# JiaoLab2021/varigraph

Measured on AMD Instinct MI355X. Metric: 150 bp reads/sec genotyped (k=27), higher is better.
Workload: dtype u64

## Files before the change

varigraph_amd/csrc/vgmi_api_table.cpp:

```cpp
#include "vgmi_ctx.h"

namespace vgapi {

void layout_image(ImageHeader& h, uint32_t k, uint64_t n_keys)
{
    memset(&h, 0, sizeof h);
    memcpy(h.magic, "VGMITBL1", 8);
    h.k = k;
    h.n_keys = n_keys;
    const bool smallk = k >= 19 && k <= 25 && n_keys <= VG_GRID_LDS_MAX_KEYS && !(getenv("VGMI_SMALLK") && getenv("VGMI_SMALLK")[0] == '0');
    const bool off_k = (getenv("VGMI_CTABLE_K") && getenv("VGMI_CTABLE_K")[0] == '0') || (getenv("VGMI_CTABLE") && getenv("VGMI_CTABLE")[0] == '0') ||
                       (getenv("VGMI_XTABLE") && getenv("VGMI_XTABLE")[0] == '0');
    const bool largek = ((k >= 19 && k <= 25 && n_keys > VG_GRID_LDS_MAX_KEYS) || ((k == 26 || k == 28) && n_keys > 0)) && n_keys < (1ULL << 31) - 16 && !off_k;
    const bool compact = (k == 27 || smallk || largek) && !getenv("VGMI_WIDE_SLOTS");
    h.slot_bytes = compact ? 8 : 16;
    uint64_t cap = 64;
    uint64_t lf_mul = compact ? 8 : 4;
    if (const char* e = getenv("VGMI_TABLE_MUL")) lf_mul = (uint64_t)atoi(e) > 1 ? (uint64_t)atoi(e) : 2;
    while (cap < lf_mul * n_keys) cap <<= 1;
    while (cap > (1ULL << 32) && cap / 2 >= 2 * n_keys) cap >>= 1;
    h.cap = cap;
    h.home_bucket_log2 = 0;
    if (k == 27 && n_keys > VG_GRID_LDS_MAX_KEYS) {
        h.home_bucket_log2 = 5;
// ... 491 lines not shown
                const uint32_t q[4] = {(uint32_t)(lo >> 24) & 0x7FFFFu, (uint32_t)(lo >> 43) & 0x7FFFFu, (uint32_t)hi & 0x7FFFFu, (uint32_t)(hi >> 19) & 0x7FFFFu};
                for (int i = 0; i < 4 && q[0] != 0; ++i) {
                    if (q[i] == 0) continue;
                    for (const uint32_t at : {q[i], flip - q[i]}) {
                        if (at >= Tp || (BKT[at] != VG_PT_NO_BUCKET && BKT[at] != (uint32_t)b)) {
                            never[b] = 1;
                            if (at < Tp) never[BKT[at]] = 1;
                            continue;
                        }
                        BKT[at] = (uint32_t)b;
                    }
                }
            }
        }
        for (uint64_t at = 0; at < Tp; ++at) {
            if (BKT[at] == VG_PT_NO_BUCKET) continue;
            for (uint32_t j = 0; j < W && at + j < Tp; ++j) NEED[BKT[at]] += vb[at + j];
        }
        for (size_t b = 0; b < n_buckets; ++b)
            if (never[b] || NEED[b] == 0) NEED[b] = 0xFFFFFFFFu;
    }
    he = hipMalloc(reinterpret_cast<void**>(&c->d_pt_index), index.size() * 8);
    if (he == hipSuccess) he = hipMalloc(reinterpret_cast<void**>(&c->d_pt_S), S.size() * 4);
    if (he == hipSuccess) he = hipMalloc(reinterpret_cast<void**>(&c->d_pt_VB), VB.size() * 4);
    const size_t pc_words = (size_t)Tp + 64, cnt_words = pt_done ? n_buckets : 0, done_words = pt_done ? (n_buckets + 31) / 32 : 0;
    const size_t live_words = pt_done ? VG_LIVE_WORDS : 0;
    const size_t sb_words = VB.size() + pc_words + cnt_words + done_words + live_words;
    if (he == hipSuccess) he = hipMalloc(reinterpret_cast<void**>(&c->d_pt_SB), sb_words * 4);
    if (pt_done) {
        if (he == hipSuccess) he = hipMalloc(reinterpret_cast<void**>(&c->d_pt_BKT), BKT.size() * 4);
        if (he == hipSuccess) he = hipMalloc(reinterpret_cast<void**>(&c->d_pt_NEED), NEED.size() * 4);
        if (he == hipSuccess) he = hipMemcpy(c->d_pt_BKT, BKT.data(), BKT.size() * 4, hipMemcpyHostToDevice);
        if (he == hipSuccess) he = hipMemcpy(c->d_pt_NEED, NEED.data(), NEED.size() * 4, hipMemcpyHostToDevice);
    }
    if (he == hipSuccess) he = hipMalloc(reinterpret_cast<void**>(&c->d_pt_SLOT), (size_t)(Tp + 64) * 4);
    if (he == hipSuccess) he = hipMemcpy(c->d_pt_index, index.data(), index.size() * 8, hipMemcpyHostToDevice);
    if (he == hipSuccess) he = hipMemcpy(c->d_pt_S, S.data(), S.size() * 4, hipMemcpyHostToDevice);
    if (he == hipSuccess) he = hipMemcpy(c->d_pt_VB, VB.data(), VB.size() * 4, hipMemcpyHostToDevice);
    if (he == hipSuccess) he = hipMemset(c->d_pt_SB, 0, sb_words * 4);
    if (he == hipSuccess) he = hipMemset(c->d_pt_SLOT, 0, (size_t)(Tp + 64) * 4);
    if (he == hipSuccess) he = hipMemcpy(c->d_pt_SLOT, slot.data(), (size_t)Tp * 4, hipMemcpyHostToDevice);
    {
        std::vector<uint32_t> place_of_slot(h.cap, 0u);
        for (uint64_t i = 0; i < n; ++i) place_of_slot[(uint32_t)P[i].y] = (uint32_t)(32 + kpos[i]);
        if (he == hipSuccess) he = hipMalloc(reinterpret_cast<void**>(&c->d_pt_PLACE), h.cap * 4);
        if (he == hipSuccess) he = hipMemcpy(c->d_pt_PLACE, place_of_slot.data(), h.cap * 4, hipMemcpyHostToDevice);
    }
    HIPCHK(c, he);
    c->pt_sb_bytes = sb_words * 4;
    if (getenv("VGMI_VERBOSE"))
        fprintf(stderr, "[vgmi] path table: %llu k-mers in %llu chains, %llu bases, %llu 12-mers with a fifth place, %llu buckets with a third 12-mer\n",
                (unsigned long long)n, (unsigned long long)chains, (unsigned long long)Tp, (unsigned long long)slow_cx, (unsigned long long)bucket_ovf);
    c->tv.pt.index = c->d_pt_index;
    c->tv.pt.S = c->d_pt_S;
    c->tv.pt.VB = c->d_pt_VB;
    c->tv.pt.SB = c->d_pt_SB;
    c->tv.pt.SLOT = c->d_pt_SLOT;
    c->tv.pt.PLACE = c->d_pt_PLACE;
    const char* pcv = getenv("VGMI_PT_POSCOUNT");
    c->tv.pt.PC = pcv && pcv[0] == '0' ? nullptr : c->d_pt_SB + VB.size();
    if (pt_done) {
        c->tv.pt.BKT = c->d_pt_BKT;
        c->tv.pt.NEED = c->d_pt_NEED;
        c->tv.pt.CNT = c->d_pt_SB + VB.size() + pc_words;
        c->tv.pt.DONE = c->tv.pt.CNT + cnt_words;
        c->tv.pt.DONE_N = c->tv.pt.DONE + done_words;
    }
    {
        const char* lv = getenv("VGMI_PT_LIVE");
        const char* lb = getenv("VGMI_PT_LIVE_BYTES");
        const unsigned long long unit = lb ? strtoull(lb, nullptr, 10) : 1ull << 30;
        c->live_unit = unit < 2048 ? 2048 : unit;
        const char* lf = getenv("VGMI_PT_LIVE_FACTOR");
        const int factor = lf ? atoi(lf) : 4;
        c->live_factor = (uint32_t)(factor < 2 ? 2 : factor > 16 ? 16 : factor);
        live_drop(c);
        if (pt_done && !(lv && lv[0] == '0') && c->tv.grid && h.grid_words_log2 == VG_GRID_LDS_WORDS_LOG2) {
            HIPCHK(c, hipMalloc(reinterpret_cast<void**>(&c->d_pt_live), (size_t)VG_LIVE_IMAGES * VG_GRID_LDS_WORDS * 4));
            for (auto& e : c->live_ev) HIPCHK(c, hipEventCreateWithFlags(&e, hipEventDisableTiming));
        }
    }
    c->tv.pt.bucket_log2 = bucket_log2;
    c->tv.pt.Tp = (uint32_t)Tp;
    return VGMI_OK;
}

}

extern "C" {


int vgmi_table_upload(vgmi_ctx* c, const uint64_t* keys, size_t n_keys, uint32_t k)
{
    if (!c) return VGMI_E_INVALID;
    if (k < 1 || k > 28) return fail(c, VGMI_E_INVALID, "k must be in 1..28 (reference assert, kmer.cpp:124)");
    if (n_keys && !keys) return fail(c, VGMI_E_INVALID, "keys is NULL");
    if (n_keys >= (1ULL << 31)) return fail(c, VGMI_E_INVALID, "too many keys");
    HIPCHK(c, hipSetDevice(c->device));
    HIPCHK(c, hipStreamSynchronize(c->stream));
    free_table(c);
    layout_image(c->hdr, k, n_keys);
    c->image_bytes = c->hdr.total_bytes;
    HIPCHK(c, hipMalloc(reinterpret_cast<void**>(&c->d_image), c->image_bytes));
    HIPCHK(c, hipMemsetAsync(c->d_image, 0, c->image_bytes, c->stream));
    HIPCHK(c, hipMemcpyAsync(c->d_image, &c->hdr, sizeof c->hdr, hipMemcpyHostToDevice, c->stream));
    HIPCHK(c, hipMemsetAsync(c->d_status, 0, 4, c->stream));
    int rc = adopt_image(c);
    if (rc) return rc;
    HIPCHK(c, launch_table_clear(c->tv, c->stream));
    uint64_t* d_keys = nullptr;
    if (n_keys) {
        HIPCHK(c, hipMalloc(reinterpret_cast<void**>(&d_keys), n_keys * 8));
        HIPCHK(c, hipMemcpyAsync(d_keys, keys, n_keys * 8, hipMemcpyHostToDevice, c->stream));
        hipError_t e = launch_table_insert(c->tv, d_keys, n_keys, k, c->d_key_slot,
                                           const_cast<uint32_t*>(c->tv.filter), const_cast<uint32_t*>(c->tv.grid),
                                           c->hdr.grid_mer == 12, c->d_status, c->stream);
        if (e != hipSuccess) { (void)hipFree(d_keys); HIPCHK(c, e); }
    }
    hipError_t e = hipStreamSynchronize(c->stream);
    if (d_keys) (void)hipFree(d_keys);
    HIPCHK(c, e);
    rc = check_status(c);
    if (rc) { free_table(c); return rc; }
    rc = build_xtable(c);
    if (rc) { free_table(c); return rc; }
    rc = build_ptable(c);
    if (rc) { free_table(c); return rc; }
    c->read_base = 0;
    return VGMI_OK;
}

int vgmi_table_lookup(vgmi_ctx* c, const uint64_t* keys, size_t n, uint32_t* index_out)
{
    if (!c || (n && (!keys || !index_out))) return VGMI_E_INVALID;
    if (!c->has_table) return fail(c, VGMI_E_STATE, "no table");
    if (n == 0) return VGMI_OK;
    HIPCHK(c, hipSetDevice(c->device));
    const TableView tv = c->tv;
    const uint64_t cap = c->hdr.cap, n_keys = c->hdr.n_keys;
    const size_t chunk = std::min<size_t>(n, (size_t)1 << 25);
    hipStream_t st = nullptr;
    uint32_t* key_of_slot = nullptr;
    uint64_t* d_keys[2] = {nullptr, nullptr};
    uint32_t* d_out[2] = {nullptr, nullptr};
    hipEvent_t done[2] = {nullptr, nullptr};
    hipError_t he = hipStreamCreateWithFlags(&st, hipStreamNonBlocking);
    if (he == hipSuccess && tv.slots8) {
        he = hipMalloc(reinterpret_cast<void**>(&key_of_slot), cap * 4);
        if (he == hipSuccess) he = hipMemsetAsync(key_of_slot, 0xFF, cap * 4, st);
        if (he == hipSuccess) he = launch_table_key_of_slot(c->d_key_slot, n_keys, key_of_slot, st);
    }
    for (int b = 0; b < 2 && he == hipSuccess; ++b) {
        he = hipMalloc(reinterpret_cast<void**>(&d_keys[b]), chunk * 8);
        if (he == hipSuccess) he = hipMalloc(reinterpret_cast<void**>(&d_out[b]), chunk * 4);
        if (he == hipSuccess) he = hipEventCreateWithFlags(&done[b], hipEventDisableTiming);
    }
    size_t at[2] = {0, 0}, len[2] = {0, 0};
    auto collect = [&](int b) {
        if (he != hipSuccess || !len[b]) return;
        he = hipEventSynchronize(done[b]);
        len[b] = 0;
    };
    int b = 0;
    for (size_t off = 0; off < n && he == hipSuccess; off += chunk, b ^= 1) {
        collect(b);
        if (he != hipSuccess) break;
// ... 168 lines not shown
```

varigraph_amd/csrc/vgmi_kernels.h:

```cpp
#ifndef VGMI_KERNELS_H
#define VGMI_KERNELS_H
#include <hip/hip_runtime.h>
#include <stdint.h>

#include "vgmi_bam_filter.h"
#include "vgmi_read_filter.h"
#include "vgmi_count_plan.h"
#include "vgmi_ctable.h"
#include "vgmi_device.h"

#ifdef VGMI_ABLATION
#define VG_DBG(x) (x)
#else
#define VG_DBG(x) 0u
#endif
uint32_t vgmi_dbg_env();

namespace vgk {

enum { K_MODE_COUNT = 0, K_MODE_KEYS = 1, K_MODE_BLOOM = 2, K_MODE_DEBIT = 3 };

#define XT_HOPS 3u
struct XTableView {
    unsigned long long* lines;
    uint32_t n_lines;
    uint32_t tag_bits;
    uint32_t id_shift;
    uint32_t* counts;
    const ulonglong2* over;
    uint32_t over_mask;
    const uint4* cb;
    uint32_t n_buckets;
    uint32_t k;
};

struct PathView {
    const unsigned long long* index;
    const uint32_t* S;
    const uint32_t* VB;
    uint32_t* SB;
    const uint32_t* SLOT;
    const uint32_t* PLACE;
    uint32_t* PC;
    const uint32_t* BKT;
    const uint32_t* NEED;
    uint32_t* CNT;
    uint32_t* DONE;
    uint32_t* DONE_N;
    uint32_t bucket_log2;
    uint32_t Tp;
};
#define VG_PT_NO_BUCKET 0xFFFFFFFFu
#define VG_LIVE_IMAGES 8u
#define VG_LIVE_WORDS (16u + 64u * 16u)
__host__ __device__ inline uint32_t vg_done_n_part(uint32_t bucket) { return 16u + ((bucket & 63u) << 4); }

struct TableView {
    VgSlot* slots;
    unsigned long long* slots8;
    uint64_t cap_mask;
    uint32_t k;
    uint32_t home_bucket_log2;
    uint32_t home_by_offset;
    const uint32_t* filter;
    uint32_t filter_words_log2;
    uint32_t filter_shift;
    const uint32_t* grid;
    uint32_t grid_words_log2;
    uint8_t* sat_dirty;
    XTableView xt;
    PathView pt;
    uint32_t* counts;
};

#define VG_BLOOM_MAX_HASH 32
struct BloomView {
    uint8_t* filter;
    uint64_t m;
    uint64_t magic;
    uint32_t n_hash;
    uint32_t seeds[VG_BLOOM_MAX_HASH];
};

struct RowParams {
    const uint8_t* bases;
    uint64_t n_bytes;
    uint64_t row_begin;
    uint64_t pair_begin;
    uint64_t row_end;
    uint64_t emit_from;
    uint32_t k;
    uint32_t dbg;
    uint32_t* status;
    const unsigned long long* n_bytes_dev;
    uint32_t tail27;
    uint32_t l1_min;
    TableView table;
    uint64_t* keys_out;
    BloomView bloom;
};

struct FqState {
    unsigned long long n_records;
    unsigned long long n_bases;
    unsigned long long consumed;
    unsigned long long packed_bytes;
    unsigned long long n_masked;
    uint32_t stopped;
    uint32_t tail_len;
    uint32_t start;
    uint32_t consumed_end;
    uint32_t n_lines, n_good, first_bad, dirty;
    unsigned long long n_seen;
    unsigned long long n_short, n_long, n_low_fraction, n_low_mean;
    uint32_t rf_dropped;
    uint32_t rf_pad;
};
struct SubParams {
    uint32_t on;
    unsigned long long seed, threshold;
};
struct FqBuffers {
    const uint8_t* raw;
    uint8_t* raw_next;
    uint8_t* packed;
    uint32_t* tile;
    uint32_t* nlpos;
    uint32_t* rec_bytes;
    uint32_t* out_off;
    uint32_t* block_sum;
    FqState* state;
    uint32_t cap_lines, tail_max;
    uint32_t min_qual;
    SubParams sub;
    vgh::ReadFilterParams rf;
};
hipError_t launch_fastq_init(FqState* st, uint32_t tail_max, hipStream_t s);
hipError_t launch_fastq_chunk(const FqBuffers& b, uint32_t n_new, hipStream_t s, const uint32_t* n_new_dev = nullptr);
hipError_t launch_scan_small(uint32_t* v, uint32_t n, uint32_t* total, hipStream_t s);

hipError_t launch_fastq_lines(const FqBuffers& b, uint32_t n_new, hipStream_t s, const uint32_t* n_new_dev = nullptr);

struct FaBuffers {
    FqBuffers q;
    unsigned long long* total;
    unsigned long long* bsum;
    uint32_t* dest;
    uint32_t* rec_d;
    uint32_t* rec_pos;
    unsigned long long* bsum_hdr;
};
// ... 273 lines not shown
```

varigraph_amd/csrc/vgmi_kernels.hip:

```cpp
#include <hip/hip_runtime.h>
#include <stdint.h>

#include "vgmi_device.h"
#include "vgmi_kernels.h"
#include "vgmi_xtable.h"

namespace vgk {

__device__ __forceinline__ uint32_t funnel(uint32_t hi, uint32_t lo, uint32_t sh)
{
    return __builtin_amdgcn_alignbit(hi, lo, sh);
}

__device__ __forceinline__ uint32_t rc_word(uint32_t x)
{
    uint32_t r = __builtin_bitreverse32(x);
    r = ((r >> 1) & 0x55555555u) | ((r & 0x55555555u) << 1);
    return ~r;
}

__device__ __forceinline__ uint64_t mod_u64(uint64_t x, uint64_t m, uint64_t magic)
{
    uint64_t q = __umul64hi(x, magic);
    uint64_t r = x - q * m;
// ... 664 lines not shown
__device__ __forceinline__ uint32_t vm_load_byte_sync(const uint8_t* ptr)
{
    uint32_t v;
    asm volatile("global_load_ubyte %0, %1, off ; VGHOT\n\ts_waitcnt vmcnt(0) ; VGHOT" : "=&v"(v) : "v"(ptr) : "memory");
    return v;
}
__device__ __forceinline__ void vm_atomic_or_sync(uint32_t* ptr, uint32_t bits)
{
    asm volatile("global_atomic_or %0, %1, off ; VGHOT\n\ts_waitcnt vmcnt(0) ; VGHOT" : : "v"(ptr), "v"(bits) : "memory");
}
__device__ __forceinline__ void vm_atomic_add_sync(uint32_t* ptr, uint32_t v)
{
    asm volatile("global_atomic_add %0, %1, off ; VGHOT\n\ts_waitcnt vmcnt(0) ; VGHOT" : : "v"(ptr), "v"(v) : "memory");
}
__device__ __forceinline__ void vm_store_byte_sync(uint8_t* ptr, uint32_t v)
{
    asm volatile("global_store_byte %0, %1, off ; VGHOT\n\ts_waitcnt vmcnt(0) ; VGHOT" : : "v"(ptr), "v"(v) : "memory");
}
template <bool COMPACT>
__device__ __forceinline__ uint4 vm_slot_value()
{
    uint4 v = make_uint4(0u, 0u, 0u, 0u);
    if (COMPACT) asm volatile("v_mov_b32 %0, v124 ; VGHOT\n\tv_mov_b32 %1, v125 ; VGHOT" : "=v"(v.x), "=v"(v.y));
    else asm volatile("v_mov_b32 %0, v124 ; VGHOT\n\tv_mov_b32 %1, v125 ; VGHOT\n\tv_mov_b32 %2, v126 ; VGHOT\n\tv_mov_b32 %3, v127 ; VGHOT"
                      : "=v"(v.x), "=v"(v.y), "=v"(v.z), "=v"(v.w));
    return v;
}
__device__ __forceinline__ uint32_t vm_atomic_old()
{
    uint32_t v;
    asm volatile("v_mov_b32 %0, v123 ; VGHOT" : "=v"(v));
    return v;
}

#define VG_ROW27 768u

#define VG_LUT27_BYTES 4096u
typedef __attribute__((address_space(3))) const uint16_t lds_u16;
typedef __attribute__((address_space(3))) const uint32_t lds_u32;

__device__ __forceinline__ void stage_lut27(uint32_t tid, uint32_t nthreads)
{
    typedef __attribute__((address_space(3))) uint16_t lds_u16_rw;
    for (uint32_t i = tid; i < 2048; i += nthreads) {
        const uint32_t set = i >> 10, b = (i >> 8) & 3u, c = vg_nt4(i & 255u);
        reinterpret_cast<lds_u16_rw*>((uintptr_t)0)[i] =
            (uint16_t)(((c & 3u) << (2 * (3 - b))) | ((c >> 2) << ((set ? 12 : 8) + b)));
    }
}

struct Addr4 { uint32_t a0, a1, a2, a3; };

#define VG_SDWA_X2(REG, B) "v_lshlrev_b32_sdwa %" #B ", %4, " REG " dst_sel:DWORD dst_unused:UNUSED_PAD src0_sel:DWORD src1_sel:BYTE_" #B " ; VGHOT\n\t"
#define VG_SDWA_ROW(REG) asm volatile(VG_SDWA_X2(REG, 0) VG_SDWA_X2(REG, 1) VG_SDWA_X2(REG, 2) VG_SDWA_X2(REG, 3) \
                                      : "=&v"(a.a0), "=&v"(a.a1), "=&v"(a.a2), "=&v"(a.a3) : "v"(one))
template <int R, int D>
__device__ __forceinline__ Addr4 lut_addr4(const uint32_t one)
{
    Addr4 a;
    if (R == 0 && D == 0) VG_SDWA_ROW("v116");
    if (R == 0 && D == 1) VG_SDWA_ROW("v117");
    if (R == 0 && D == 2) VG_SDWA_ROW("v118");
    if (R == 1 && D == 0) VG_SDWA_ROW("v120");
    if (R == 1 && D == 1) VG_SDWA_ROW("v121");
    if (R == 1 && D == 2) VG_SDWA_ROW("v122");
    return a;
}

template <int R, int D>
__device__ __forceinline__ Addr4 luts_addr4(const uint32_t one)
{
    Addr4 a;
    if (R == 0 && D == 0) VG_SDWA_ROW("v116");
    if (R == 0 && D == 1) VG_SDWA_ROW("v117");
    if (R == 0 && D == 2) VG_SDWA_ROW("v118");
    if (R == 0 && D == 3) VG_SDWA_ROW("v119");
    if (R == 1 && D == 0) VG_SDWA_ROW("v120");
    if (R == 1 && D == 1) VG_SDWA_ROW("v121");
    if (R == 1 && D == 2) VG_SDWA_ROW("v122");
    if (R == 1 && D == 3) VG_SDWA_ROW("v123");
    return a;
}

template <int SET>
__device__ __forceinline__ uint32_t encode4(const Addr4& a)
{
    const uint32_t e0 = *reinterpret_cast<lds_u16*>((uintptr_t)(a.a0 + SET * 2048u));
    const uint32_t e1 = *reinterpret_cast<lds_u16*>((uintptr_t)(a.a1 + SET * 2048u + 512u));
    const uint32_t e2 = *reinterpret_cast<lds_u16*>((uintptr_t)(a.a2 + SET * 2048u + 1024u));
    uint32_t e3 = *reinterpret_cast<lds_u16*>((uintptr_t)(a.a3 + SET * 2048u + 1536u));
    asm("" : "+v"(e3));
    return e0 | e1 | e2 | e3;
}

template <bool LDS_BM, bool COMPACT>
__global__ __launch_bounds__(LDS_BM ? 1024 : 256) void count27_kernel(RowParams p)
{
    constexpr uint32_t MASK_HI = (1u << (2 * 27 - 32)) - 1;
    extern __shared__ __attribute__((aligned(16))) uint8_t smem[];
    const uint32_t tid = threadIdx.x;
    const uint32_t lane = tid & 63u;
    const uint32_t wave = tid >> 6;
    const uint32_t nwaves = blockDim.x >> 6;

    typedef uint32_t u32x4 __attribute__((ext_vector_type(4)));
    typedef __attribute__((address_space(3))) u32x4 lds_u4_rw;
    typedef __attribute__((address_space(3))) uint64_t lds_u64_rw;
    const uint32_t wave_u = (uint32_t)__builtin_amdgcn_readfirstlane((int)wave);
    const uint32_t rings0 = VG_LUT27_BYTES + (LDS_BM ? VG_GRID_LDS_WORDS * 4u : 0u);
    const uint32_t runs_base = rings0 + wave_u * (VG_RUNQ * 16u);
    const uint32_t req_base = rings0 + nwaves * (VG_RUNQ * 16u) + wave_u * (VG_REQ * 8u);
    stage_lut27(tid, blockDim.x);
    if (LDS_BM) {
        const uint4* src = reinterpret_cast<const uint4*>(p.table.grid);
        uint4* dst = reinterpret_cast<uint4*>(smem + VG_LUT27_BYTES);
        for (uint32_t i = tid; i < VG_GRID_LDS_WORDS / 4; i += blockDim.x) dst[i] = src[i];
    }
    __syncthreads();
    const uint32_t* g_grid = p.table.grid;
    const uint32_t gwl = LDS_BM ? VG_GRID_LDS_WORDS_LOG2 : p.table.grid_words_log2;
    VgSlot* const slots = p.table.slots;
    unsigned long long* const slots8 = p.table.slots8;
    uint32_t* const counts = p.table.counts;
    const uint64_t cap_mask = p.table.cap_mask;
    const uint32_t hb_log2 = p.table.home_bucket_log2;
    const bool hb_off = p.table.home_by_offset != 0;

    const uint64_t total_pairs = p.n_bytes_dev ? *p.n_bytes_dev / (2 * VG_ROW27) : p.row_end >> 1;
    const uint64_t total_waves = (uint64_t)gridDim.x * nwaves;
    const uint64_t ppw = (total_pairs + total_waves - 1) / total_waves;
    const uint64_t gw = (uint64_t)blockIdx.x * nwaves + wave_u;
    const uint64_t r0v = gw * ppw;
    const uint64_t r1v = r0v + ppw < total_pairs ? r0v + ppw : total_pairs;
    const uint64_t r0 = ((uint64_t)(uint32_t)__builtin_amdgcn_readfirstlane((int)(r0v >> 32)) << 32) |
                        (uint32_t)__builtin_amdgcn_readfirstlane((int)(uint32_t)r0v);
    const uint64_t r1 = ((uint64_t)(uint32_t)__builtin_amdgcn_readfirstlane((int)(r1v >> 32)) << 32) |
                        (uint32_t)__builtin_amdgcn_readfirstlane((int)(uint32_t)r1v);
    if (r0 >= r1) return;
    uint32_t one;
    asm volatile("v_mov_b32 %0, 1" : "=v"(one));
    const uint32_t lane_off = lane * 12u;
    const uint8_t* const bases = p.bases;

    uint32_t pr1_be = 0, pr2_be = 0, pr3_be = 0, pr1_inv = 0xFFFu, pr2_inv = 0xFFFu, pr3_inv = 0xFFFu;
    const uint64_t rs = r0 > 0 ? r0 - 1 : r0;

    uint32_t n_after_row = 0;
    uint32_t n_after_slot = 2;
    uint64_t b_canon = 0, b_slot = 0;
    bool b_active = false;
    uint64_t p_slot = 0;
    bool p_bumped = false;

    const uint32_t my_run = lane / 12u, my_win = lane % 12u;
    const uint32_t my_sh = 2 * (11 - my_win), my_vbit = 12 + my_win;
    uint32_t run_head = 0, run_n = 0, req_head = 0, req_n = 0;
    auto ring_slot = [](uint32_t pos) -> uint32_t {
        const uint32_t w = pos - VG_RUNQ;
        return w < pos ? w : pos;
    };

    auto probe_issue = [&](bool act, uint64_t kmer, uint64_t dist) __attribute__((always_inline)) {
        const uint64_t rc = vg_revcomp(kmer, 27);
        const uint64_t canon = kmer < rc ? kmer : rc;
        b_canon = canon | (dist << 54);
        const uint64_t home = (!LDS_BM && hb_log2) ? vg_thash_local(canon, canon == kmer ? rc : kmer, hb_log2, hb_off) : vg_thash(canon);
// ... 174 lines not shown
        const uint32_t iB1 = lane >= 1 ? b1_inv : a1_inv, iB2 = lane >= 2 ? b2_inv : a2_inv, iB3 = lane >= 3 ? b3_inv : a3_inv;
        pr1_be = b1_be; pr2_be = b2_be; pr3_be = b3_be; pr1_inv = b1_inv; pr2_inv = b2_inv; pr3_inv = b3_inv;
        if (it < n_warm) continue;

        {
            const uint32_t adjA = invA & ((invA << 1) | (iA1 >> 11));
            const uint32_t adjB = invB & ((invB << 1) | (iB1 >> 11));
            if (__builtin_expect(__ballot((adjA | adjB) != 0) != 0, 0)) {
                empty_read_check(adjA, cur);
                empty_read_check(adjB, cur + VG_ROW27);
            }
        }

        const RowScan sa = scan_probe(beA, invA, beA1, beA2, beA3, iA1, iA2, iA3);
        const RowScan sb = scan_probe(beB, invB, beB1, beB2, beB3, iB1, iB2, iB3);
        const uint64_t ballA = __builtin_amdgcn_ballot_w64(sa.ok16 && (sa.gw32 & sa.gm) == sa.gm && sa.vm != 0);
        const uint64_t ballB = __builtin_amdgcn_ballot_w64(sb.ok16 && (sb.gw32 & sb.gm) == sb.gm && sb.vm != 0);
        const uint32_t nA = (uint32_t)__builtin_popcountll(ballA), nB = (uint32_t)__builtin_popcountll(ballB);
        if (VG_DBG(p.dbg) & 1u) continue;
        enqueue(sa, ballA, run_head + run_n);
        run_n += nA;
        while (run_n + nB > VG_RUNQ) drain_step();
        enqueue(sb, ballB, run_head + run_n);
        run_n += nB;
        if (run_n >= VG_RUN_BATCH || req_n >= 32u) drain_step();
        while (run_n >= 3 * VG_RUN_BATCH || req_n >= 48u) drain_step();
    }
    do {
        drain_step();
    } while (run_n != 0 || req_n != 0 || __builtin_amdgcn_ballot_w64(b_active) != 0);
    vm_wait_imm<0>();
}

#define VG_ROW27S 1024u
#define VG_RUN_BATCH_S 4u

template <bool PT, uint32_t K = 27>
__global__ __launch_bounds__(1024) void count27s_kernel(RowParams p)
{
    static_assert(K == 27 || (PT && K >= 19 && K <= 25), "count27s_kernel: k = 27, or the path-table form for k = 19 .. 25 (a run of k + 7 bases is two words)");
    constexpr uint32_t MASK_HI = (1u << (2 * K - 32)) - 1;
    extern __shared__ __attribute__((aligned(16))) uint8_t smem[];
    const uint32_t tid = threadIdx.x;
    const uint32_t lane = tid & 63u;
    const uint32_t wave = tid >> 6;
    const uint32_t nwaves = blockDim.x >> 6;
    typedef uint32_t u32x4 __attribute__((ext_vector_type(4)));
    typedef __attribute__((address_space(3))) u32x4 lds_u4_rw;
    typedef __attribute__((address_space(3))) uint64_t lds_u64_rw;
    const uint32_t wave_u = (uint32_t)__builtin_amdgcn_readfirstlane((int)wave);
    const uint32_t rings0 = VG_LUT27_BYTES + VG_GRID_LDS_WORDS * 4u;
    const uint32_t runs_base = rings0 + wave_u * (VG_RUNQ * 16u);
    const uint32_t req_base = rings0 + nwaves * (VG_RUNQ * 16u) + wave_u * (VG_REQ * 8u);
    stage_lut27(tid, blockDim.x);
    {
        const uint4* src = reinterpret_cast<const uint4*>(p.table.grid);
        uint4* dst = reinterpret_cast<uint4*>(smem + VG_LUT27_BYTES);
        for (uint32_t i = tid; i < VG_GRID_LDS_WORDS / 4; i += blockDim.x) dst[i] = src[i];
    }
    __syncthreads();
    unsigned long long* const slots8 = p.table.slots8;
    uint32_t* const counts = p.table.counts;
    const uint64_t cap_mask = p.table.cap_mask;

    const uint64_t total_pairs = p.n_bytes_dev ? *p.n_bytes_dev / (2 * VG_ROW27S) : p.row_end >> 1;
    const uint64_t pair_begin = p.n_bytes_dev ? 0u : p.pair_begin;
    const uint64_t total_waves = (uint64_t)gridDim.x * nwaves;
    const uint64_t ppw = (total_pairs - pair_begin + total_waves - 1) / total_waves;
    const uint64_t gw = (uint64_t)blockIdx.x * nwaves + wave_u;
    const uint64_t r0v = pair_begin + gw * ppw;
    const uint64_t r1v = r0v + ppw < total_pairs ? r0v + ppw : total_pairs;
    const uint64_t r0 = ((uint64_t)(uint32_t)__builtin_amdgcn_readfirstlane((int)(r0v >> 32)) << 32) |
                        (uint32_t)__builtin_amdgcn_readfirstlane((int)(uint32_t)r0v);
    const uint64_t r1 = ((uint64_t)(uint32_t)__builtin_amdgcn_readfirstlane((int)(r1v >> 32)) << 32) |
                        (uint32_t)__builtin_amdgcn_readfirstlane((int)(uint32_t)r1v);
    if (r0 >= r1) return;
    uint32_t one;
    asm volatile("v_mov_b32 %0, 1" : "=v"(one));
    const uint32_t lane_off = lane * 16u;
    const uint8_t* const bases = p.bases;

    uint32_t pr1_be = 0, pr2_be = 0, pr1_inv = 0xFFFFu, pr2_inv = 0xFFFFu;
    const uint64_t rs = r0 > 0 ? r0 - 1 : r0;

    uint32_t n_after_row = 0, n_after_slot = 2;
    uint64_t b_canon = 0, b_slot = 0;
    bool b_active = false;
    uint64_t p_slot = 0;
    bool p_bumped = false;

    const uint32_t my_run = lane >> 4, my_win = lane & 15u;
    const uint32_t my_sh = 2 * (15 - my_win);
    uint32_t run_head = 0, run_n = 0, req_head = 0, req_n = 0;
    auto ring_slot = [](uint32_t pos) -> uint32_t {
        const uint32_t w = pos - VG_RUNQ;
        return w < pos ? w : pos;
    };

    auto probe_issue = [&](bool act, uint64_t kmer, uint64_t dist) __attribute__((always_inline)) {
        const uint64_t rc = vg_revcomp(kmer, K);
        const uint64_t canon = kmer < rc ? kmer : rc;
        b_canon = canon | (dist << 54);
        b_slot = (vg_thash(canon) + dist) & cap_mask;
        b_active = act;
        if (act) vms_load_slot(&slots8[b_slot]);
        ++n_after_row;
        n_after_slot = 0;
    };
    constexpr uint32_t RQ = 112;
    const uint32_t rq_base = rings0 + wave_u * (VG_RUNQ * 16u + VG_REQ * 8u);
    auto rq_wrap = [](uint32_t pos) -> uint32_t { return pos >= RQ ? pos - RQ : pos; };
    const unsigned long long* const pt_index = p.table.pt.index;
    const uint32_t* const ptS = p.table.pt.S;
    const uint32_t* const ptVB = p.table.pt.VB;
    uint32_t* const ptSB = p.table.pt.SB;
    const uint32_t* const ptSLOT = p.table.pt.SLOT;
    uint32_t* const ptPC = p.table.pt.PC;
    const uint32_t* const ptBKT = p.table.pt.BKT;
    const uint32_t* const ptNEED = p.table.pt.NEED;
    uint32_t* const ptCNT = p.table.pt.CNT;
    uint32_t* const ptDONE_N = p.table.pt.DONE_N;
    uint32_t* const ptDONE = p.table.pt.DONE;
    const uint32_t pt_Tp = p.table.pt.Tp, pt_bshift = 32u - p.table.pt.bucket_log2;
    const uint32_t l1_min = (uint32_t)__builtin_amdgcn_readfirstlane((int)p.l1_min);
    uint32_t n_after_idx = 8, n_after_seq = 8;
    u32x4 l1_run = {0u, 0u, 0u, 0u};
    uint32_t l1_n = 0, l1_phase = 0;
    uint32_t pl[4] = {0u, 0u, 0u, 0u};
    bool l1_slow = false;
    uint32_t l1_done_bit = 0;
    auto hot = [&](uint32_t k) __attribute__((always_inline)) {
        n_after_row += k;
        n_after_idx += k;
        n_after_seq += k;
    };
    auto set_saturated = [&](uint32_t pos, uint32_t mir) __attribute__((always_inline)) -> uint32_t {
        const uint32_t a = vm_atomic_or_ret_sync(ptSB + (pos >> 5), 1u << (pos & 31u));
        const uint32_t b = vm_atomic_or_ret_sync(ptSB + (mir >> 5), 1u << (mir & 31u));
        return ((~a >> (pos & 31u)) & 1u) | (((~b >> (mir & 31u)) & 1u) << 1);
    };
    auto done_events = [&](uint32_t fired, uint32_t pos) __attribute__((always_inline)) {
        constexpr uint32_t W = K == 27 ? 16u : 8u;
        uint64_t ev = __builtin_amdgcn_ballot_w64(fired != 0);
        while (ev != 0) {
            const uint32_t src = (uint32_t)__builtin_ctzll(ev);
            ev &= ev - 1;
            const uint32_t f = (uint32_t)__builtin_amdgcn_readlane((int)fired, (int)src), x0 = (uint32_t)__builtin_amdgcn_readlane((int)pos, (int)src);
            const uint32_t x = lane < 16u ? x0 : pt_Tp - K - x0;
            if (lane < 32u && (lane & 15u) < W && ((f >> (lane >> 4)) & 1u)) pt_done_step<true>(ptBKT, ptNEED, ptCNT, ptDONE, ptDONE_N, x - (lane & 15u));
        }
    };
    auto slow_count = [&](uint32_t klo, uint32_t khi, uint32_t& fired, uint32_t& at) __attribute__((always_inline)) {
        const uint64_t kmer = (uint64_t)khi << 32 | klo, rc = vg_revcomp(kmer, K);
        if (!(K & 1u) && kmer == rc) return;
        const uint64_t canon = kmer < rc ? kmer : rc;
        uint64_t sl = vg_thash(canon) & cap_mask;
        for (;;) {
            const uint4 v = vm_load_slot_sync<true>(&slots8[sl]);
            const uint64_t c = ((uint64_t)v.y << 32) | v.x;
            if (c == VG_EMPTY) break;
            if ((c & VG_SLOT_KMER_MASK) == canon) {
                if (!(c & VG_SLOT_SAT) && vm_atomic_inc_sync(&counts[sl], one) == 254u) {
                    vm_atomic_or_sync(reinterpret_cast<uint32_t*>(&slots8[sl]) + 1, (uint32_t)(VG_SLOT_SAT >> 32));
                    vm_store_byte_sync(p.table.sat_dirty + (sl >> VG_SAT_REGION_LOG2), 1u);
                    const uint32_t pos = vm_load_dword_sync(p.table.pt.PLACE + sl);
                    if (pos != 0u) {
// ... 307 lines not shown
    auto make_room = [&]() __attribute__((always_inline)) {
        while (l1_phase != 0) l1_advance();
        resolve_issue();
    };

    struct RowScan { uint32_t W0, W1, W2, vm, gm, gw32, cm; };
    auto scan_probe = [&](uint32_t be, uint32_t inv, uint32_t be1, uint32_t be2, uint32_t i1, uint32_t i2) __attribute__((always_inline)) -> RowScan {
        RowScan r;
        r.W0 = be;
        r.W1 = be1;
        r.W2 = be2;
        const uint32_t B = (i2 >> 5) | (i1 << 11);
        const uint32_t a = (inv << 1) & 0xFFFFu;
        const uint32_t bad_b = B ? (0xFFFFFFFFu >> __builtin_clz(B)) : 0u;
        r.vm = ~(a | (0u - a) | bad_b) & 0xFFFFu;
        const uint32_t mer = be1 & 0xFFFFFFu, rcm = vg_revcomp12(mer);
        const uint32_t cm = mer < rcm ? mer : rcm;
        r.cm = cm | (mer <= rcm ? 1u << 24 : 0u);
        const uint32_t h1 = vg_mul24(cm, 0x9E3779u), h2 = vg_mul24(cm, 0x85EBCBu);
        r.gm = (1u << (h2 >> 27)) | (1u << ((h2 >> 22) & 31u)) | (1u << ((h2 >> 17) & 31u));
        r.gw32 = *reinterpret_cast<lds_u32*>((uintptr_t)(((h1 >> (32 - VG_GRID_LDS_WORDS_LOG2)) << 2) + VG_LUT27_BYTES));
        return r;
    };
    auto enqueue = [&](const RowScan& r, uint64_t ball, uint32_t tail) __attribute__((always_inline)) {
        if (__builtin_amdgcn_inverse_ballot_w64(ball)) {
            const uint32_t d0 = funnel(r.W1, r.W0, 2);
            const uint32_t d1 = funnel(r.W2, r.W1, 2);
            const uint32_t d2 = r.W2 >> 2;
            const uint32_t pos = __builtin_amdgcn_mbcnt_hi((uint32_t)(ball >> 32), __builtin_amdgcn_mbcnt_lo((uint32_t)ball, tail));
            if (PT)
                *reinterpret_cast<lds_u4_rw*>((uintptr_t)(rq_base + rq_wrap(pos) * 16u)) =
                    u32x4{d0, d1, (d2 & 0xFFFFFu) | (r.vm << 20), r.cm | ((r.vm >> 12) << 28)};
            else
                *reinterpret_cast<lds_u4_rw*>((uintptr_t)(runs_base + ring_slot(pos) * 16u)) = u32x4{d0, d1, d2, r.vm};
        }
    };
    auto scan_probe_k = [&](uint32_t be, uint32_t inv, uint32_t be1, uint32_t be2, uint32_t i1, uint32_t i2, uint32_t H) __attribute__((always_inline)) -> RowScan {
        RowScan r;
        r.W0 = be;
        r.W1 = be1;
        r.W2 = be2;
        const uint32_t g = 32u + 8u * H;
        const uint64_t I = (uint64_t)i2 | (uint64_t)i1 << 16 | (uint64_t)inv << 32;
        const uint32_t B = (uint32_t)(I >> (g + 1u - K)) & ((1u << K) - 1u);
        const uint32_t a = (uint32_t)(I >> g) & 0xFEu;
        const uint32_t bad_b = B ? (0xFFFFFFFFu >> __builtin_clz(B)) : 0u;
        r.vm = ~(a | (0u - a) | bad_b) & 0xFFu;
        const uint32_t mer = funnel(be1, be, 30u - 16u * H) & 0xFFFFFFu, rcm = vg_revcomp12(mer);
        const uint32_t cm = mer < rcm ? mer : rcm;
        r.cm = cm | (mer <= rcm ? 1u << 24 : 0u);
        const uint32_t h1 = vg_mul24(cm, 0x9E3779u), h2 = vg_mul24(cm, 0x85EBCBu);
        r.gm = (1u << (h2 >> 27)) | (1u << ((h2 >> 22) & 31u)) | (1u << ((h2 >> 17) & 31u));
        r.gw32 = *reinterpret_cast<lds_u32*>((uintptr_t)(((h1 >> (32 - VG_GRID_LDS_WORDS_LOG2)) << 2) + VG_LUT27_BYTES));
        return r;
    };
    auto enqueue_k = [&](const RowScan& r, uint64_t ball, uint32_t tail, uint32_t H) __attribute__((always_inline)) {
        if (__builtin_amdgcn_inverse_ballot_w64(ball)) {
            const uint32_t sh = 16u - 16u * H;
            const uint32_t d0 = funnel(r.W1, r.W0, sh);
            const uint32_t d1 = funnel(r.W2, r.W1, sh) & ((K + 7u == 32u) ? 0xFFFFFFFFu : (1u << ((2u * (K + 7u) - 32u) & 31u)) - 1u);
            const uint32_t pos = __builtin_amdgcn_mbcnt_hi((uint32_t)(ball >> 32), __builtin_amdgcn_mbcnt_lo((uint32_t)ball, tail));
            *reinterpret_cast<lds_u4_rw*>((uintptr_t)(rq_base + rq_wrap(pos) * 16u)) = u32x4{d0, d1, r.vm, r.cm};
        }
    };
    auto empty_read_check = [&](uint32_t adj, const uint8_t* row) __attribute__((always_inline)) {
        if (adj) {
            const uint64_t base_off = (uint64_t)(row - bases) + lane_off;
            for (uint32_t t = 0; t < 16; ++t) {
                if (!((adj >> t) & 1u)) continue;
                const uint64_t o = base_off + t;
                if (vm_load_byte_sync(bases + o) == '\n' && (o == 0 || vm_load_byte_sync(bases + o - 1) == '\n'))
                    vm_atomic_or_sync(p.status, 1u);
            }
        }
    };

    const uint32_t n_it = (uint32_t)(r1 - rs), n_warm = (uint32_t)(r0 - rs);
    const uint8_t* rowp = bases + rs * (2 * VG_ROW27S);
    vms_load_row<0>(rowp + lane_off);
    vms_load_row<1>(rowp + VG_ROW27S + lane_off);
    for (uint32_t it = 0; it < n_it; ++it) {
        if (PT) vm_wait4(n_after_row);
        else vm_wait(n_after_row);
        const Addr4 a0 = luts_addr4<0, 0>(one), a1 = luts_addr4<0, 1>(one), a2 = luts_addr4<0, 2>(one), a3 = luts_addr4<0, 3>(one);
        const Addr4 c0 = luts_addr4<1, 0>(one), c1 = luts_addr4<1, 1>(one), c2 = luts_addr4<1, 2>(one), c3 = luts_addr4<1, 3>(one);
        const uint8_t* const cur = rowp;
        if (it + 1 < n_it) rowp += 2 * VG_ROW27S;
        vms_load_row<0>(rowp + lane_off);
        vms_load_row<1>(rowp + VG_ROW27S + lane_off);
        n_after_row = 0;
        n_after_slot += 2;
        if (PT) {
            n_after_idx += 2;
            n_after_seq += 2;
        } else if (run_n >= VG_RUN_BATCH_S || req_n >= 32u) drain_step();

        const uint32_t g0 = encode4<0>(a0), g1 = encode4<1>(a1), g2 = encode4<0>(a2), g3 = encode4<1>(a3);
        const uint32_t h0 = encode4<0>(c0), h1 = encode4<1>(c1), h2 = encode4<0>(c2), h3 = encode4<1>(c3);
        const uint32_t beA = __builtin_amdgcn_perm(__builtin_amdgcn_perm(g0, g1, 0x0c0c0400u), __builtin_amdgcn_perm(g2, g3, 0x0c0c0400u), 0x05040100u);
        const uint32_t invA = (((g0 | g1) >> 8) & 0xFFu) | ((g2 | g3) & 0xFF00u);
        const uint32_t beB = __builtin_amdgcn_perm(__builtin_amdgcn_perm(h0, h1, 0x0c0c0400u), __builtin_amdgcn_perm(h2, h3, 0x0c0c0400u), 0x05040100u);
        const uint32_t invB = (((h0 | h1) >> 8) & 0xFFu) | ((h2 | h3) & 0xFF00u);
        auto ror1 = [](uint32_t v) __attribute__((always_inline)) -> uint32_t {
            return (uint32_t)__builtin_amdgcn_mov_dpp((int)v, 0x13C , 0xF, 0xF, false);
        };
        const uint32_t a1_be = ror1(beA), a1_inv = ror1(invA), b1_be = ror1(beB), b1_inv = ror1(invB);
        const uint32_t a2_be = ror1(a1_be), a2_inv = ror1(a1_inv), b2_be = ror1(b1_be), b2_inv = ror1(b1_inv);
        const uint32_t beA1 = lane >= 1 ? a1_be : pr1_be, beA2 = lane >= 2 ? a2_be : pr2_be;
        const uint32_t iA1 = lane >= 1 ? a1_inv : pr1_inv, iA2 = lane >= 2 ? a2_inv : pr2_inv;
        const uint32_t beB1 = lane >= 1 ? b1_be : a1_be, beB2 = lane >= 2 ? b2_be : a2_be;
        const uint32_t iB1 = lane >= 1 ? b1_inv : a1_inv, iB2 = lane >= 2 ? b2_inv : a2_inv;
        pr1_be = b1_be; pr2_be = b2_be; pr1_inv = b1_inv; pr2_inv = b2_inv;
        if (it < n_warm) continue;

        {
            const uint32_t adjA = invA & ((invA << 1) | (iA1 >> 15));
            const uint32_t adjB = invB & ((invB << 1) | (iB1 >> 15));
            if (__builtin_expect(__ballot(((adjA | adjB) & 0xFFFFu) != 0) != 0, 0)) {
                empty_read_check(adjA & 0xFFFFu, cur);
                empty_read_check(adjB & 0xFFFFu, cur + VG_ROW27S);
            }
        }

        if constexpr (K != 27) {
#pragma unroll 1
            for (uint32_t h = 0; h < 4u; ++h) {
                const bool second = h >= 2u;
                const RowScan sc = scan_probe_k(second ? beB : beA, second ? invB : invA, second ? beB1 : beA1, second ? beB2 : beA2,
                                                second ? iB1 : iA1, second ? iB2 : iA2, h & 1u);
                const uint64_t ball = __builtin_amdgcn_ballot_w64((sc.gw32 & sc.gm) == sc.gm && sc.vm != 0);
                if (VG_DBG(p.dbg) & 1u) continue;
                const uint32_t nh = (uint32_t)__builtin_popcountll(ball);
                if (run_n + nh > RQ) make_room();
                enqueue_k(sc, ball, run_head + run_n, h & 1u);
                run_n += nh;
            }
            l1_advance();
            if (l1_phase == 0 && run_n >= l1_min) resolve_issue();
            continue;
        }
        const RowScan sa = scan_probe(beA, invA, beA1, beA2, iA1, iA2);
        const RowScan sb = scan_probe(beB, invB, beB1, beB2, iB1, iB2);
        const uint64_t ballA = __builtin_amdgcn_ballot_w64((sa.gw32 & sa.gm) == sa.gm && sa.vm != 0);
        const uint64_t ballB = __builtin_amdgcn_ballot_w64((sb.gw32 & sb.gm) == sb.gm && sb.vm != 0);
        const uint32_t nA = (uint32_t)__builtin_popcountll(ballA), nB = (uint32_t)__builtin_popcountll(ballB);
        if (VG_DBG(p.dbg) & 1u) continue;
        if (PT) {
            if (run_n + nA > RQ) make_room();
            enqueue(sa, ballA, run_head + run_n);
            run_n += nA;
            if (run_n + nB > RQ) make_room();
            enqueue(sb, ballB, run_head + run_n);
            run_n += nB;
            l1_advance();
            if (l1_phase == 0 && run_n >= l1_min) resolve_issue();
            continue;
        }
        enqueue(sa, ballA, run_head + run_n);
        run_n += nA;
        while (run_n + nB > VG_RUNQ) drain_step();
        enqueue(sb, ballB, run_head + run_n);
        run_n += nB;
        if (run_n >= VG_RUN_BATCH_S || req_n >= 32u) drain_step();
        while (run_n >= 3 * VG_RUN_BATCH_S || req_n >= 48u) drain_step();
    }
    if (PT) {
        while (run_n != 0 || l1_phase != 0) {
            while (l1_phase != 0) l1_advance();
            if (run_n != 0) resolve_issue();
        }
    } else {
        do {
            drain_step();
        } while (run_n != 0 || req_n != 0 || __builtin_amdgcn_ballot_w64(b_active) != 0);
    }
    vm_wait_imm<0>();
}

#define VG_SEQ_LDS 16384u


template <int MODE, bool DEV = false>
__global__ __launch_bounds__(256) void seq_kernel(RowParams p, const uint64_t* read_off, uint64_t n_reads, const unsigned long long* n_reads_dev = nullptr)
{
    __shared__ __attribute__((aligned(16))) uint8_t s_text[4][VG_SEQ_LDS];
    const uint32_t lane = threadIdx.x & 63u, wave = threadIdx.x >> 6;
    uint64_t r = (uint64_t)blockIdx.x * blockDim.x + threadIdx.x;
    uint64_t n_bytes = p.n_bytes, emit_from = p.emit_from;
    if constexpr (DEV) {
        n_reads = *n_reads_dev < n_reads ? *n_reads_dev : n_reads;
        n_bytes = *p.n_bytes_dev;
        emit_from = vg_row_split(p.tail27, n_bytes).emit_from;
        if (p.tail27) {
            if (emit_from >= n_bytes) return;
            uint64_t lo = 0, hi = n_reads;
            while (lo < hi) {
                const uint64_t mid = (lo + hi) >> 1;
                if (read_off[mid + 1] <= emit_from) lo = mid + 1;
                else hi = mid;
            }
            r += lo;
        }
    }
    const uint64_t r_first = r - lane;
    bool staged = false;
    uint64_t stage_base = 0;
    if (r_first < n_reads) {
        const uint64_t r_last = r_first + 64 < n_reads ? r_first + 64 : n_reads;
        const uint64_t b = read_off[r_first] & ~15ULL, e = read_off[r_last];
        if (MODE == MODE_COUNT && e <= emit_from) return;
        if (e - b <= VG_SEQ_LDS && e <= ((n_bytes + 15) & ~15ULL)) {
            for (uint64_t o = b + lane * 16u; o < e; o += 1024)
                *reinterpret_cast<uint4*>(&s_text[wave][o - b]) = load_chunk(p.bases, n_bytes, o);
            staged = true;
            stage_base = b;
        }
    }
    __builtin_amdgcn_fence(__ATOMIC_ACQ_REL, "wavefront");
    __builtin_amdgcn_wave_barrier();
    if (r >= n_reads) return;
    const uint64_t s = read_off[r];
    const uint64_t e = read_off[r + 1] - (MODE == MODE_BLOOM ? 0 : 1);
    if (e <= s) {
        atomicOr(p.status, 1u);
        return;
    }
    const uint32_t K = p.k;
    const uint64_t mask = (1ULL << (2 * K)) - 1, shift1 = 2 * (uint64_t)(K - 1);
    uint64_t fwd = 0, rc = 0;
    uint32_t l = 0;
    for (uint64_t i = s; i < e; ++i) {
        const uint32_t c = vg_nt4(staged ? s_text[wave][i - stage_base] : p.bases[i]);
        uint64_t out = ~0ULL;
        if (c < 4) {
            fwd = (fwd << 2 | c) & mask;
            rc = (rc >> 2) | (uint64_t)(3u ^ c) << shift1;
            if (fwd != rc) {
                ++l;
                if (l >= K) {
                    const uint64_t canon = fwd < rc ? fwd : rc;
// ... 639 lines not shown
```

Measured before the change: 33.31 billion.

## Add probe-first fast path for k=27 path-table scan skipping full encode

For the PT k=27 loop, each wave first runs a cheap own-lane grid-filter probe on the high 24-bit part of each k-mer and only builds the full encoded k-mers, neighbour shifts and scan_probe when some lane passes. Otherwise it saves the raw row bytes as halo state and lazily reconstructs them in the next iteration that does go long. This aims to cut LDS lookups and DPP shuffles on rows with no candidate hits, at the cost of extra control flow, carry state and a second probe. It can be disabled with VGMI_PT_PROBE_FIRST=0.

```diff
diff --git a/varigraph_amd/csrc/vgmi_api_table.cpp b/varigraph_amd/csrc/vgmi_api_table.cpp
--- a/varigraph_amd/csrc/vgmi_api_table.cpp
+++ b/varigraph_amd/csrc/vgmi_api_table.cpp
@@ -597,6 +597,8 @@
     }
     c->tv.pt.bucket_log2 = bucket_log2;
     c->tv.pt.Tp = (uint32_t)Tp;
+    const char* pfv = getenv("VGMI_PT_PROBE_FIRST");
+    c->tv.probe_first = pfv && pfv[0] == '0' ? 0u : 1u;
     return VGMI_OK;
 }
 
diff --git a/varigraph_amd/csrc/vgmi_kernels.h b/varigraph_amd/csrc/vgmi_kernels.h
--- a/varigraph_amd/csrc/vgmi_kernels.h
+++ b/varigraph_amd/csrc/vgmi_kernels.h
@@ -67,6 +67,7 @@
     uint32_t filter_shift;
     const uint32_t* grid;
     uint32_t grid_words_log2;
+    uint32_t probe_first;
     uint8_t* sat_dirty;
     XTableView xt;
     PathView pt;
diff --git a/varigraph_amd/csrc/vgmi_kernels.hip b/varigraph_amd/csrc/vgmi_kernels.hip
--- a/varigraph_amd/csrc/vgmi_kernels.hip
+++ b/varigraph_amd/csrc/vgmi_kernels.hip
@@ -770,6 +770,25 @@
     return a;
 }
 
+template <int R>
+__device__ __forceinline__ uint32_t luts_raw0()
+{
+    uint32_t v;
+    if (R == 0) asm volatile("v_mov_b32 %0, v116 ; VGHOT" : "=v"(v));
+    else asm volatile("v_mov_b32 %0, v120 ; VGHOT" : "=v"(v));
+    return v;
+}
+__device__ __forceinline__ Addr4 lut_addr4_of(const uint32_t raw, const uint32_t one)
+{
+    Addr4 a;
+    asm("v_lshlrev_b32_sdwa %0, %4, %5 dst_sel:DWORD dst_unused:UNUSED_PAD src0_sel:DWORD src1_sel:BYTE_0\n\t"
+        "v_lshlrev_b32_sdwa %1, %4, %5 dst_sel:DWORD dst_unused:UNUSED_PAD src0_sel:DWORD src1_sel:BYTE_1\n\t"
+        "v_lshlrev_b32_sdwa %2, %4, %5 dst_sel:DWORD dst_unused:UNUSED_PAD src0_sel:DWORD src1_sel:BYTE_2\n\t"
+        "v_lshlrev_b32_sdwa %3, %4, %5 dst_sel:DWORD dst_unused:UNUSED_PAD src0_sel:DWORD src1_sel:BYTE_3"
+        : "=&v"(a.a0), "=&v"(a.a1), "=&v"(a.a2), "=&v"(a.a3) : "v"(one), "v"(raw));
+    return a;
+}
+
 template <int SET>
 __device__ __forceinline__ uint32_t encode4(const Addr4& a)
 {
@@ -1110,6 +1129,9 @@
 
     uint32_t pr1_be = 0, pr2_be = 0, pr1_inv = 0xFFFFu, pr2_inv = 0xFFFFu;
     const uint64_t rs = r0 > 0 ? r0 - 1 : r0;
+    [[maybe_unused]] bool halo_raw = false, carry_long = false;
+    [[maybe_unused]] uint32_t cv63 = 0xFFFFFFFFu;
+    [[maybe_unused]] const bool probe_first = p.table.probe_first != 0;
 
     uint32_t n_after_row = 0, n_after_slot = 2;
     uint64_t b_canon = 0, b_slot = 0;
@@ -1583,6 +1605,99 @@
     for (uint32_t it = 0; it < n_it; ++it) {
         if (PT) vm_wait4(n_after_row);
         else vm_wait(n_after_row);
+        if constexpr (PT && K == 27) {
+            const Addr4 a1 = luts_addr4<0, 1>(one), a2 = luts_addr4<0, 2>(one), a3 = luts_addr4<0, 3>(one);
+            const Addr4 c1 = luts_addr4<1, 1>(one), c2 = luts_addr4<1, 2>(one), c3 = luts_addr4<1, 3>(one);
+            const uint32_t rawA = luts_raw0<0>(), rawB = luts_raw0<1>();
+            const uint8_t* const cur = rowp;
+            if (it + 1 < n_it) rowp += 2 * VG_ROW27S;
+            vms_load_row<0>(rowp + lane_off);
+            vms_load_row<1>(rowp + VG_ROW27S + lane_off);
+            n_after_row = 0;
+            n_after_slot += 2;
+            n_after_idx += 2;
+            n_after_seq += 2;
+            auto ror1 = [](uint32_t v) __attribute__((always_inline)) -> uint32_t {
+                return (uint32_t)__builtin_amdgcn_mov_dpp((int)v, 0x13C , 0xF, 0xF, false);
+            };
+            const uint32_t g1 = encode4<1>(a1), g2 = encode4<0>(a2), g3 = encode4<1>(a3);
+            const uint32_t h1 = encode4<1>(c1), h2 = encode4<0>(c2), h3 = encode4<1>(c3);
+            const uint32_t merA = __builtin_amdgcn_perm(g1, __builtin_amdgcn_perm(g2, g3, 0x0c0c0400u), 0x0c040100u);
+            const uint32_t merB = __builtin_amdgcn_perm(h1, __builtin_amdgcn_perm(h2, h3, 0x0c0c0400u), 0x0c040100u);
+            const uint32_t invA_hi = ((g1 >> 8) & 0xF0u) | ((g2 | g3) & 0xFF00u);
+            const uint32_t invB_hi = ((h1 >> 8) & 0xF0u) | ((h2 | h3) & 0xFF00u);
+            const uint32_t cv = (invA_hi | ((~rawA & 0x40404040u) ? 0xFu : 0u)) | ((invB_hi | ((~rawB & 0x40404040u) ? 0xFu : 0u)) << 16);
+            const uint32_t cv_last = (uint32_t)__builtin_amdgcn_readlane((int)cv, 63);
+            const uint32_t cv_halo = (cv63 >> 16) | (cv_last << 16);
+            cv63 = cv_last;
+            if (it < n_warm) {
+                pr1_be = rawB; pr2_be = merB; pr1_inv = invB_hi;
+                halo_raw = true;
+                carry_long = true;
+                continue;
+            }
+            {
+                const uint32_t nb = lane >= 1 ? ror1(cv) : cv_halo;
+                const uint32_t adj = cv & (((cv << 1) & 0xFFFEFFFEu) | ((nb >> 15) & 0x00010001u));
+                if (__builtin_expect(__ballot(adj != 0) != 0, 0)) {
+                    empty_read_check(adj & 0xFFFFu, cur);
+                    empty_read_check(adj >> 16, cur + VG_ROW27S);
+                }
+            }
+            bool go_long = carry_long || !probe_first;
+            if (probe_first) {
+                auto own_pass = [&](uint32_t mer) __attribute__((always_inline)) -> bool {
+                    const uint32_t rcm = vg_revcomp12(mer);
+                    const uint32_t cm = mer < rcm ? mer : rcm;
+                    const uint32_t q1 = vg_mul24(cm, 0x9E3779u), q2 = vg_mul24(cm, 0x85EBCBu);
+                    const uint32_t gm = (1u << (q2 >> 27)) | (1u << ((q2 >> 22) & 31u)) | (1u << ((q2 >> 17) & 31u));
+                    const uint32_t gw32 = *reinterpret_cast<lds_u32*>((uintptr_t)(((q1 >> (32 - VG_GRID_LDS_WORDS_LOG2)) << 2) + VG_LUT27_BYTES));
+                    return (gw32 & gm) == gm;
+                };
+                const uint64_t ownA = __builtin_amdgcn_ballot_w64(own_pass(merA));
+                const uint64_t ownB = __builtin_amdgcn_ballot_w64(own_pass(merB));
+                go_long = go_long || (ownA | ownB) != 0;
+                carry_long = (ownB >> 63) != 0;
+            }
+            if (go_long) {
+                if (halo_raw) {
+                    const uint32_t p0 = encode4<0>(lut_addr4_of(pr1_be, one));
+                    const uint32_t pbe = __builtin_amdgcn_perm(p0, pr2_be, 0x04020100u), pinv = ((p0 >> 8) & 0xFu) | pr1_inv;
+                    pr1_be = ror1(pbe); pr1_inv = ror1(pinv);
+                    pr2_be = ror1(pr1_be); pr2_inv = ror1(pr1_inv);
+                }
+                const uint32_t g0 = encode4<0>(lut_addr4_of(rawA, one)), h0 = encode4<0>(lut_addr4_of(rawB, one));
+                const uint32_t beA = __builtin_amdgcn_perm(g0, merA, 0x04020100u), invA = ((g0 >> 8) & 0xFu) | invA_hi;
+                const uint32_t beB = __builtin_amdgcn_perm(h0, merB, 0x04020100u), invB = ((h0 >> 8) & 0xFu) | invB_hi;
+                const uint32_t a1_be = ror1(beA), a1_inv = ror1(invA), b1_be = ror1(beB), b1_inv = ror1(invB);
+                const uint32_t a2_be = ror1(a1_be), a2_inv = ror1(a1_inv), b2_be = ror1(b1_be), b2_inv = ror1(b1_inv);
+                const uint32_t beA1 = lane >= 1 ? a1_be : pr1_be, beA2 = lane >= 2 ? a2_be : pr2_be;
+                const uint32_t iA1 = lane >= 1 ? a1_inv : pr1_inv, iA2 = lane >= 2 ? a2_inv : pr2_inv;
+                const uint32_t beB1 = lane >= 1 ? b1_be : a1_be, beB2 = lane >= 2 ? b2_be : a2_be;
+                const uint32_t iB1 = lane >= 1 ? b1_inv : a1_inv, iB2 = lane >= 2 ? b2_inv : a2_inv;
+                pr1_be = b1_be; pr2_be = b2_be; pr1_inv = b1_inv; pr2_inv = b2_inv;
+                halo_raw = false;
+                const RowScan sa = scan_probe(beA, invA, beA1, beA2, iA1, iA2);
+                const RowScan sb = scan_probe(beB, invB, beB1, beB2, iB1, iB2);
+                const uint64_t ballA = __builtin_amdgcn_ballot_w64((sa.gw32 & sa.gm) == sa.gm && sa.vm != 0);
+                const uint64_t ballB = __builtin_amdgcn_ballot_w64((sb.gw32 & sb.gm) == sb.gm && sb.vm != 0);
+                const uint32_t nA = (uint32_t)__builtin_popcountll(ballA), nB = (uint32_t)__builtin_popcountll(ballB);
+                if (VG_DBG(p.dbg) & 1u) continue;
+                if (run_n + nA > RQ) make_room();
+                enqueue(sa, ballA, run_head + run_n);
+                run_n += nA;
+                if (run_n + nB > RQ) make_room();
+                enqueue(sb, ballB, run_head + run_n);
+                run_n += nB;
+            } else {
+                pr1_be = rawB; pr2_be = merB; pr1_inv = invB_hi;
+                halo_raw = true;
+                if (VG_DBG(p.dbg) & 1u) continue;
+            }
+            l1_advance();
+            if (l1_phase == 0 && run_n >= l1_min) resolve_issue();
+            continue;
+        }
         const Addr4 a0 = luts_addr4<0, 0>(one), a1 = luts_addr4<0, 1>(one), a2 = luts_addr4<0, 2>(one), a3 = luts_addr4<0, 3>(one);
         const Addr4 c0 = luts_addr4<1, 0>(one), c1 = luts_addr4<1, 1>(one), c2 = luts_addr4<1, 2>(one), c3 = luts_addr4<1, 3>(one);
         const uint8_t* const cur = rowp;
@@ -1646,17 +1761,6 @@
         const uint64_t ballB = __builtin_amdgcn_ballot_w64((sb.gw32 & sb.gm) == sb.gm && sb.vm != 0);
         const uint32_t nA = (uint32_t)__builtin_popcountll(ballA), nB = (uint32_t)__builtin_popcountll(ballB);
         if (VG_DBG(p.dbg) & 1u) continue;
-        if (PT) {
-            if (run_n + nA > RQ) make_room();
-            enqueue(sa, ballA, run_head + run_n);
-            run_n += nA;
-            if (run_n + nB > RQ) make_room();
-            enqueue(sb, ballB, run_head + run_n);
-            run_n += nB;
-            l1_advance();
-            if (l1_phase == 0 && run_n >= l1_min) resolve_issue();
-            continue;
-        }
         enqueue(sa, ballA, run_head + run_n);
         run_n += nA;
         while (run_n + nB > VG_RUNQ) drain_step();
```

Result: slower. 13.42 billion (-59.7%).
